# wirrell/SPART-python

Hardware: AMD Instinct MI355X
Metric: SPART spectra/sec (R_TOC+R_TOA+L_TOA) at batch 1M; achieved HBM GB/s vs peak (higher is better)
Workload: dtype f32

## Files before the change

### spart-python_amd/csrc/spart_kernels.h

```cpp
#pragma once

#include <type_traits>

#include "spart_math.h"

namespace spart {

constexpr int TILE = 256;
constexpr int NTILE = 8;
constexpr int NTILE_FULL = 9;
constexpr int MAX_NB = NWLS;

__device__ __forceinline__ void xcd_map(unsigned b, int& tile, int64_t& ck) {
  tile = (int)((b >> 3) & 7u);
  ck = (int64_t)(b >> 6) * 8 + (b & 7u);
}
inline unsigned xcd_grid(int64_t nchunk) { return (unsigned)(((nchunk + 7) / 8) * 64); }

struct ParamPtrs {
  const double* p[NPARAM];
  const double* rho_th;
  const double* tau_th;
  const double* lidf;
  int nlayers;
// ... 13 lines not shown
  const int si = threadIdx.x & 31, i0 = threadIdx.x >> 5;
  const unsigned lane_off = ((unsigned)i0 * (unsigned)Bp + (unsigned)si) * (unsigned)sizeof(T);
  if (si < nsub) {
#pragma unroll
    for (int k = 0; k < NCONST / 8; ++k) {
      const T* row = blk + (int64_t)(8 * k) * Bp;
      lds_c[si * NCONST + i0 + 8 * k] = *reinterpret_cast<const T*>(reinterpret_cast<const char*>(row) + lane_off);
    }
  }
}

template <typename T, int SUB>
__device__ __forceinline__ void stage_fetch(T (&r)[NCONST * SUB / TILE], const T* __restrict__ blk, int64_t Bp, int nsub) {
  constexpr int RP = TILE / SUB;
  static_assert(TILE % SUB == 0 && NCONST % RP == 0, "whole passes");
  const int si = threadIdx.x % SUB, i0 = threadIdx.x / SUB;
  const unsigned lane_off = ((unsigned)i0 * (unsigned)Bp + (unsigned)si) * (unsigned)sizeof(T);
  if (si < nsub) {
#pragma unroll
    for (int k = 0; k < NCONST / RP; ++k) {
      const T* row = blk + (int64_t)(RP * k) * Bp;
      r[k] = *reinterpret_cast<const T*>(reinterpret_cast<const char*>(row) + lane_off);
    }
  }
}
template <typename T, int SUB>
__device__ __forceinline__ void stage_put(T* lds_c, const T (&r)[NCONST * SUB / TILE], int nsub) {
  constexpr int RP = TILE / SUB;
  const int si = threadIdx.x % SUB, i0 = threadIdx.x / SUB;
  if (si < nsub) {
#pragma unroll
    for (int k = 0; k < NCONST / RP; ++k) lds_c[si * NCONST + i0 + RP * k] = r[k];
  }
}

struct PreludeStore {
  float* cstF;
  double* cstD;
  double* atm;
  int64_t Bp, s;
  __device__ __forceinline__ void c(int i, double v) const {
    if (cstF) cstF[i * Bp + s] = (float)v;
    if (cstD) cstD[i * Bp + s] = v;
  }
  __device__ __forceinline__ void a(int i, double v) const {
    if (atm) atm[i * Bp + s] = v;
  }
  __device__ __forceinline__ void l(int, double) const {}
};

constexpr int PRELUDE_SIMD_WAVES = 3;
template <bool FAST, bool USER = false>
__global__ __launch_bounds__(256, PRELUDE_SIMD_WAVES) void k_prelude(ParamPtrs pp, int mask, int64_t B, int64_t Bp, float* __restrict__ cstF,
                                                 double* __restrict__ cstD, double* __restrict__ atm) {
  const int64_t base = (int64_t)blockIdx.x * blockDim.x;
  int64_t s = base + threadIdx.x;
  if (!FAST && (mask & PRE_CANOPY) && !(USER && pp.lidf)) {
    constexpr int NB = 32;
    __shared__ int cnt[NB], start[NB];
    __shared__ unsigned char perm[256];
    const int t = threadIdx.x;
    int bucket = NB - 1;
    if (s < B) {
      const double key = ::fabs(pp.p[16][s]) + ::fabs(pp.p[17][s]);
      const double q = key * (NB / 1.0);
      bucket = !(q < (double)(NB - 1)) ? NB - 1 : (q > 0.0 ? (int)q : 0);
    }
    if (t < NB) cnt[t] = 0;
    __syncthreads();
    const int pos = atomicAdd(&cnt[bucket], 1);
    __syncthreads();
    if (t == 0) {
      int acc = 0;
      for (int i = 0; i < NB; ++i) { start[i] = acc; acc += cnt[i]; }
    }
    __syncthreads();
    perm[start[bucket] + pos] = (unsigned char)t;
    __syncthreads();
    s = base + perm[t];
  }
  if (s >= B) return;
  double rho_th = pp.rho_th ? pp.rho_th[s] : 0.01;
  double tau_th = pp.tau_th ? pp.tau_th[s] : 0.01;
  PreludeStore out{cstF, cstD, atm, Bp, s};
  if (USER)
    sample_prelude_to<FAST, true>([&pp, s](int i) { return pp.p[i] ? pp.p[i][s] : 0.0; }, rho_th, tau_th, mask, out,
                                  pp.lidf ? pp.lidf + s * NLINCL : nullptr, pp.nlayers);
  else
    sample_prelude_to<FAST>([&pp, s](int i) { return pp.p[i] ? pp.p[i][s] : 0.0; }, rho_th, tau_th, mask, out);
}

static __global__ __launch_bounds__(256) void k_lidf(const double* __restrict__ a, const double* __restrict__ b, int64_t B,
                                              double* __restrict__ lidf) {
  int64_t s = (int64_t)blockIdx.x * blockDim.x + threadIdx.x;
  if (s >= B) return;
  double li[NLINCL];
  leaf_angles(a[s], b[s], li);
#pragma unroll
  for (int i = 0; i < NLINCL; ++i) lidf[s * NLINCL + i] = li[i];
}

template <typename T> __device__ __forceinline__ BandTab<T> load_tab(const T* __restrict__ tab, int i) {
  BandTab<T> t;
  t.kab = tab[TAB_KAB * NWL + i];
  t.kca = tab[TAB_KCA * NWL + i];
  t.kdm = tab[TAB_KDM * NWL + i];
  t.kw = tab[TAB_KW * NWL + i];
  t.ks = tab[TAB_KS * NWL + i];
  t.kant = tab[TAB_KANT * NWL + i];
  t.kcbc = tab[TAB_CBC * NWL + i];
  t.kprot = tab[TAB_PROT * NWL + i];
  t.talf = tab[TAB_TALF * NWL + i];
  t.t12 = tab[TAB_T12 * NWL + i];
  t.t21 = tab[TAB_T21 * NWL + i];
  t.g0 = tab[TAB_GSV0 * NWL + i];
  t.g1 = tab[TAB_GSV1 * NWL + i];
  t.g2 = tab[TAB_GSV2 * NWL + i];
  t.cbac = tab[TAB_CBAC * NWL + i];
  t.pw = tab[TAB_PW * NWL + i];
  t.rw = tab[TAB_RW * NWL + i];
  return t;
}

template <typename T, typename C> __device__ __forceinline__ CanopyPar<T> load_canopy(const C& c) {
  CanopyPar<T> cp;
  cp.sob = c[C_SOB]; cp.sof = c[C_SOF];
  cp.hbf = c[C_HBF]; cp.ks = c[C_KS]; cp.ko = c[C_KO]; cp.lai = c[C_LAI]; cp.lai2 = c[C_LAI2];
  cp.tss = c[C_TSS]; cp.too = c[C_TOO]; cp.Z = c[C_Z]; cp.hot = c[C_HOT]; cp.pso2w = c[C_PSO2W];
  return cp;
}

template <bool NT = false, typename T> __device__ __forceinline__ void store_row(T* row, unsigned byte_off, T v) {
  T* p = reinterpret_cast<T*>(reinterpret_cast<char*>(row) + byte_off);
  if (NT) __builtin_nontemporal_store(v, p);
  else *p = v;
}
inline bool nt_ok(int pitch_elems, size_t elem_size) { return ((size_t)pitch_elems * elem_size) % 128 == 0; }

template <typename T> struct MatPtrs {
  T *leaf_refl, *leaf_tran, *leaf_kchl, *soil_refl, *soil_dry, *rso, *rdo, *rsd, *rdd;
  const T* rdry_in;
  int pf, po;
};

template <typename T, int MAT, int FULL, bool NT = false>
__global__ __launch_bounds__(TILE, (sizeof(T) == 8 ? 3 : 1))
void k_bands(const T* __restrict__ tab, const T* __restrict__ cst, int64_t Bp, int64_t B, int chunk, MatPtrs<T> mat,
             T* __restrict__ bandsum) {
  int tile;
  int64_t ck;
  xcd_map(blockIdx.x, tile, ck);
  if (ck * chunk >= B) return;
  if (sizeof(T) == 8) stage_f64_tables();
  const int band = tile * TILE + threadIdx.x;
  const bool active = band < NEVAL;
  const bool thermal = band == NWL;
  const int ti = band < NWL ? band : NWL - 1;
  const BandTab<T> tb = load_tab(tab, ti);
  const int64_t s0 = ck * chunk;
  const int64_t s1 = (s0 + chunk < B) ? s0 + chunk : B;
  T sum_so = T(0), sum_do = T(0), sum_sd = T(0), sum_dd = T(0);
  unsigned off_f = (unsigned)band * (unsigned)sizeof(T), off_o = off_f;
  if (MAT) {
    const int64_t b0f = s0 * mat.pf, b0o = s0 * mat.po;
    if (mat.leaf_refl) mat.leaf_refl += b0f;
    if (mat.leaf_tran) mat.leaf_tran += b0f;
    if (mat.soil_refl) mat.soil_refl += b0f;
    if (mat.rso) mat.rso += b0f;
    if (mat.rdo) mat.rdo += b0f;
    if (mat.rsd) mat.rsd += b0f;
    if (mat.rdd) mat.rdd += b0f;
    if (mat.leaf_kchl) mat.leaf_kchl += b0o;
    if (mat.soil_dry) mat.soil_dry += b0o;
  }
  constexpr int SUB = 32;
  constexpr bool HOIST_FILM = sizeof(T) == 8;
  constexpr bool PINGPONG = sizeof(T) == 4 && MAT == 0;
  __shared__ __attribute__((aligned(16))) T lds_all[(PINGPONG ? 2 : 1) * SUB * NCONST + (PINGPONG ? NCONST : 0)];
  T stg[NCONST * SUB / TILE];
  int cur = 0;
  if (PINGPONG) {
    const int n0 = (int)((s1 - s0 < SUB) ? (s1 - s0) : SUB);
    stage_fetch<T, SUB>(stg, cst + s0, Bp, n0);
    stage_put<T, SUB>(lds_all, stg, n0);
    __syncthreads();
  }
  for (int64_t sb = s0; sb < s1; sb += SUB) {
  const int nsub = (int)((s1 - sb < SUB) ? (s1 - sb) : SUB);
  T* const lds_c = lds_all + cur * (SUB * NCONST);
  const int nnext = (int)((s1 - sb - SUB < SUB) ? (s1 - sb - SUB) : SUB);
  if (PINGPONG) {
    if (nnext > 0) stage_fetch<T, SUB>(stg, cst + sb + SUB, Bp, nnext);
  } else {
    __syncthreads();
    stage_constants<T>(lds_c, cst + sb, Bp, nsub);
    __syncthreads();
  }
  bool film_same = false;
  T tw1s = T(0);
  if (HOIST_FILM) {
    const int l = threadIdx.x & 63;
    const T f0 = lds_c[C_FILM2L];
    const T fl = lds_c[(l < nsub ? l : 0) * NCONST + C_FILM2L];
    film_same = __all(fl == f0) != 0;
    if (film_same) tw1s = soil_tw1<T>(tb, f0);
  }
  constexpr bool AHEAD = MAT == 0 && sizeof(T) == 4;
  static_assert(AHEAD == PINGPONG, "the look-ahead read relies on the padding of lds_all");
  int lane0 = 0;
  if (AHEAD) {
    SPART_KEEP_BRANCH(lane0);
    lane0 &= ~3;
  }
  T lc[9];
#pragma unroll
  for (int i = 0; i < 9; ++i) lc[i] = lds_c[i];
  constexpr bool COMMON = sizeof(T) == 4 && MAT == 0 && FULL == 1;
  bool common = false;
  T tw1c = T(0);
  if (COMMON) {
    const int l = threadIdx.x & 63;
    const T* cl = lds_c + (l < nsub ? l : 0) * NCONST;
    common = __all(cl[C_FILM2L] == lds_c[C_FILM2L] && cl[C_CBC] == T(0) && cl[C_PROT] == T(0)) != 0;
    if (common) tw1c = soil_tw1<T>(tb, lds_c[C_FILM2L]);
  }
  constexpr bool VOTES = sizeof(T) == 4 && MAT == 0;
  unsigned long long j2_mask = ~0ull;
  if constexpr (VOTES) {
    const int l = threadIdx.x & 63;
    const T* cl = lds_c + (l < nsub ? l : 0) * NCONST;
    j2_mask = __ballot(sail_j2_possible(cl[C_KSL], cl[C_LAI]) || sail_j2_possible(cl[C_KOL], cl[C_LAI]));
  }
  auto sample_loop = [&](auto common_tag) __attribute__((always_inline)) {
  constexpr bool FAST = decltype(common_tag)::value;
  for (int si = 0; si < nsub; ++si) {
    const int64_t s = sb + si;
    const T* c = lds_c + si * NCONST + lane0;
    T refl, tran, absb, K;
    static_assert(C_CAB == 0 && C_NM1 == 8, "lc[] = constants 0..8 in leaf_band's argument order");
    if (!AHEAD) {
#pragma unroll
      for (int i = 0; i < 9; ++i) lc[i] = c[i];
    }
    leaf_band<T, !FAST>(tb, lc[0], lc[1], lc[2], lc[3], lc[4], lc[5], lc[6], lc[7], lc[8], refl, tran, absb, K);
    if (AHEAD) {
      const T* cn = c + NCONST;
#pragma unroll
      for (int i = 0; i < 9; ++i) lc[i] = cn[i];
    }
    T rho = refl, tau = tran, ab = absb;
    if (tile == NTILE - 1) {
      rho = thermal ? c[C_RHO_TH] : refl;
      tau = thermal ? c[C_TAU_TH] : tran;
      ab = thermal ? (T(1) - c[C_RHO_TH] - c[C_TAU_TH]) : absb;
    }
    if (MAT && active) {
      if (mat.leaf_refl) store_row<NT>(mat.leaf_refl, off_f, rho);
      if (mat.leaf_tran) store_row<NT>(mat.leaf_tran, off_f, tau);
      if (!thermal && mat.leaf_kchl) store_row<NT>(mat.leaf_kchl, off_o, (K > T(0)) ? divx(c[C_CAB] * tb.kab, K) : T(0));
    }
    const CanopyPar<T> cp = load_canopy<T>(c);
    const CanopyCore<T> core = canopy_core_l<T>(cp, rho, tau, ab, c[C_KSL], c[C_KOL], !VOTES || ((j2_mask >> si) & 1) != 0);
    T rdry = (MAT == 2) ? mat.rdry_in[s * mat.po + ti] : soil_dry<T>(tb, c[C_F1], c[C_F2], c[C_F3]);
    T fm[7] = {c[C_FM0], c[C_FM1], c[C_FM2], c[C_FM3], c[C_FM4], c[C_FM5], c[C_FM6]};
    T rwet, tw1;
    if (FAST) tw1 = tw1c;
    else if (HOIST_FILM && film_same) tw1 = tw1s;
    else tw1 = soil_tw1<T>(tb, c[C_FILM2L]);
    soil_band_tw<T>(tb, rdry, c[C_WET], fm, c[C_FMSUM], tw1, rwet);
    if (MAT && active) {
      if (mat.soil_refl) store_row<NT>(mat.soil_refl, off_f, rwet);
      if (!thermal && mat.soil_dry) store_row<NT>(mat.soil_dry, off_o, rdry);
    }
    constexpr bool SUM_ONLY = FULL == 1 && MAT == 0 && sizeof(T) == 4;
    T rso, rdo, rsd, rdd;
    if (SUM_ONLY) {
      sum_so += canopy_soil_sum<T>(cp, core, rwet, c[C_TSTO]);
    } else {
      canopy_soil<T>(cp, core, rwet, rso, rdo, rsd, rdd);
      if (FULL == 2) {
        sum_so += rso; sum_do += rdo; sum_sd += rsd; sum_dd += rdd;
      } else if (FULL == 1) {
        sum_so += (rso + rdo) + (rsd + rdd);
      }
    }
    if (MAT) {
      if (active) {
        if (mat.rso) store_row<NT>(mat.rso, off_f, rso);
        if (mat.rdo) store_row<NT>(mat.rdo, off_f, rdo);
        if (mat.rsd) store_row<NT>(mat.rsd, off_f, rsd);
        if (mat.rdd) store_row<NT>(mat.rdd, off_f, rdd);
      }
      constexpr int TH_WAVE = (NWL % TILE) / 64, TH_LANE = (NWL % TILE) % 64;
      if (tile == NTILE - 1 && (int)(threadIdx.x >> 6) == TH_WAVE) {
        const unsigned pad = off_f + (unsigned)((TH_LANE + 1) * (int)sizeof(T));
        T* arrs[7] = {mat.leaf_refl, mat.leaf_tran, mat.soil_refl, mat.rso, mat.rdo, mat.rsd, mat.rdd};
        const T vals[7] = {rho, tau, rwet, rso, rdo, rsd, rdd};
        const int l = threadIdx.x & 63;
#pragma unroll
        for (int q = 0; q < 7; ++q) {
          const T v = __shfl(vals[q], TH_LANE, 64);
          if (arrs[q]) {
            store_row(arrs[q], pad, v);
            store_row(arrs[q], pad + 64u * (unsigned)sizeof(T), v);
            if (l < NWLT - 1 - 128) store_row(arrs[q], pad + 128u * (unsigned)sizeof(T), v);
          }
        }
      }
      off_f += (unsigned)mat.pf * (unsigned)sizeof(T);
      off_o += (unsigned)mat.po * (unsigned)sizeof(T);
    }
  }
  };
  if constexpr (COMMON) {
    if (common) sample_loop(std::true_type{});
    else sample_loop(std::false_type{});
  } else {
    sample_loop(std::false_type{});
  }
  if (PINGPONG) {
    if (nnext > 0) stage_put<T, SUB>(lds_all + (cur ^ 1) * (SUB * NCONST), stg, nnext);
    __syncthreads();
    cur ^= 1;
  }
  }
  if (FULL == 2) {
    T* bs = bandsum + (ck * (NTILE * TILE) + band) * 4;
    bs[0] = sum_so; bs[1] = sum_do; bs[2] = sum_sd; bs[3] = sum_dd;
  } else if (FULL == 1) {
    bandsum[ck * (NTILE * TILE) + band] = sum_so;
  }
}

template <typename T> struct LdsCol {
  const T* p;
  __device__ __forceinline__ T operator[](int i) const { return p[i * 64]; }
};


constexpr int COL_WAVES = 4;
constexpr int COLUMNS_SIMD_WAVES = 4;

template <typename TG, typename TO, typename TR>
__global__ __launch_bounds__(64 * COL_WAVES, COLUMNS_SIMD_WAVES) void k_columns(
    const TG* __restrict__ tab, const TG* __restrict__ cst, const double* __restrict__ atm, int64_t Bp,
    const int* __restrict__ band0, const int* __restrict__ band1, const double* __restrict__ frac,
    const double* __restrict__ coef, const double* __restrict__ econv, int nb, const TR* __restrict__ rdry_in, int po, int64_t B,
    TO* __restrict__ R_TOC, TO* __restrict__ R_TOA, TO* __restrict__ L_TOA, TO* __restrict__ o_rsoil, TO* __restrict__ o_La) {
  __shared__ TG lds_c[NCONST_USED * 64];
  __shared__ double lds_a[NATM_USED * 64];
  __shared__ double lds_k[COL_WAVES * 64];
  if (sizeof(TG) == 8) stage_f64_tables();
  const int lane = threadIdx.x & 63;
  const int wave = __builtin_amdgcn_readfirstlane((int)(threadIdx.x >> 6));
  const int64_t s0 = (int64_t)blockIdx.x * 64;
  const int64_t s = s0 + lane;
  const bool ok = s < B;
  const int64_t sc = ok ? s : B - 1;
  for (int i = wave; i < NCONST_USED; i += COL_WAVES) lds_c[i * 64 + lane] = cst[(int64_t)i * Bp + sc];
  for (int i = wave; i < NATM_USED; i += COL_WAVES) lds_a[i * 64 + lane] = atm[(int64_t)i * Bp + sc];
  __syncthreads();
  const LdsCol<TG> c{lds_c + lane};
  const LdsCol<double> a{lds_a + lane};
  const bool want_soil = o_rsoil != nullptr;
  for (int j = wave; j < nb; j += COL_WAVES) {
    const int b0 = band0[j], b1 = band1[j];
    const double f = frac[j];
    const double kv = coef[(size_t)(lane < NCOEF ? lane : NCOEF - 1) * nb + j];
    double y0[5], y1[5];
#pragma unroll 1
    for (int e = 0; e < 2; ++e) {
      if (e == 1 && b1 == b0) break;
      const int band = e ? b1 : b0;
      const bool thermal = band == NWL;
      const int ti = band < NWL ? band : NWL - 1;
      const BandTab<TG> tb = load_tab(tab, ti);
      TG refl, tran, absb, K;
      leaf_band<TG>(tb, c[C_CAB], c[C_CCA], c[C_CDM], c[C_CW], c[C_CS], c[C_CANT], c[C_CBC], c[C_PROT], c[C_NM1], refl,
                    tran, absb, K);
      const TG rho = thermal ? c[C_RHO_TH] : refl;
      const TG tau = thermal ? c[C_TAU_TH] : tran;
      const TG ab = thermal ? (TG(1) - c[C_RHO_TH] - c[C_TAU_TH]) : absb;
      const CanopyPar<TG> cp = load_canopy<TG>(c);
      const CanopyCore<TG> core = canopy_core<TG>(cp, rho, tau, ab);
      const TG rdry = rdry_in ? (TG)rdry_in[sc * po + ti] : soil_dry<TG>(tb, c[C_F1], c[C_F2], c[C_F3]);
      TG fm[7] = {c[C_FM0], c[C_FM1], c[C_FM2], c[C_FM3], c[C_FM4], c[C_FM5], c[C_FM6]};
      TG rwet;
      soil_band<TG>(tb, rdry, c[C_WET], fm, c[C_FMSUM], c[C_FILM2L], rwet);
      TG rso, rdo, rsd, rdd;
      canopy_soil<TG>(cp, core, rwet, rso, rdo, rsd, rdd);
      const double v[5] = {(double)rso, (double)rdo, (double)rsd, (double)rdd, (double)rwet};
#pragma unroll
      for (int q = 0; q < 5; ++q) {
        if (e == 0) y0[q] = v[q];
        y1[q] = v[q];
      }
    }
    double v[5];
#pragma unroll
    for (int q = 0; q < 5; ++q) v[q] = y0[q] + (y1[q] - y0[q]) * f;
    double* kw = lds_k + wave * 64;
    kw[lane] = kv;
    __builtin_amdgcn_fence(__ATOMIC_RELEASE, "wavefront");
    __builtin_amdgcn_wave_barrier();
    __builtin_amdgcn_fence(__ATOMIC_ACQUIRE, "wavefront");
    const SmacOut so = smac_band_c(a, [kw](int r) { return kw[r]; });
    const double La = a[A_LAF] * econv[j];
    double rtoc, rtoa, ltoa;
    toc_to_toa(so, v[0], v[1], v[3], v[2], La, rtoc, rtoa, ltoa);
    if (ok) {
      const int64_t o = s * nb + j;
      R_TOC[o] = (TO)rtoc;
      R_TOA[o] = (TO)rtoa;
      L_TOA[o] = (TO)ltoa;
      if (want_soil) o_rsoil[o] = (TO)v[4];
      if (o_La) o_La[o] = (TO)La;
    }
  }
}

template <typename TO, typename TR>
__global__ __launch_bounds__(64 * COL_WAVES, COLUMNS_SIMD_WAVES) void k_columns_srf(
    const double* __restrict__ tab, const double* __restrict__ cst, const double* __restrict__ atm, int64_t Bp,
    const int* __restrict__ deal, const int* __restrict__ sup_start, const int* __restrict__ sup_ev,
    const double* __restrict__ sup_q, const double* __restrict__ sup_Q, const double* __restrict__ coef,
    const double* __restrict__ econv, int nb, const TR* __restrict__ rdry_in, int po, int64_t B, TO* __restrict__ R_TOC,
    TO* __restrict__ R_TOA, TO* __restrict__ L_TOA, TO* __restrict__ o_rso, TO* __restrict__ o_rdo, TO* __restrict__ o_rsd,
    TO* __restrict__ o_rdd) {
  __shared__ double lds_c[NCONST_USED * 64];
  __shared__ double lds_a[NATM_USED * 64];
  __shared__ double lds_k[COL_WAVES * 64];
  stage_f64_tables();
  const int lane = threadIdx.x & 63;
  const int wave = __builtin_amdgcn_readfirstlane((int)(threadIdx.x >> 6));
  const int64_t s = (int64_t)blockIdx.x * 64 + lane;
  const bool ok = s < B;
  const int64_t sc = ok ? s : B - 1;
  for (int i = wave; i < NCONST_USED; i += COL_WAVES) lds_c[i * 64 + lane] = cst[(int64_t)i * Bp + sc];
  for (int i = wave; i < NATM_USED; i += COL_WAVES) lds_a[i * 64 + lane] = atm[(int64_t)i * Bp + sc];
  __syncthreads();
  const int j = deal[blockIdx.y * COL_WAVES + wave];
  if (j < 0) return;
  const int e0 = sup_start[j], e1 = sup_start[j + 1];
  double acc_so = 0.0, acc_do = 0.0, acc_sd = 0.0, acc_dd = 0.0;
#pragma unroll 1
  for (int e = e0; e < e1; ++e) {
    int lo = lane;
    SPART_KEEP_BRANCH(lo);
    const LdsCol<double> c{lds_c + lo};
    const int band = sup_ev[e];
    const double q = sup_q[e];
    const bool thermal = band == NWL;
    const int ti = band < NWL ? band : NWL - 1;
    const BandTab<double> tb = load_tab(tab, ti);
    double refl, tran, absb, K;
    leaf_band<double>(tb, c[C_CAB], c[C_CCA], c[C_CDM], c[C_CW], c[C_CS], c[C_CANT], c[C_CBC], c[C_PROT], c[C_NM1], refl,
                      tran, absb, K);
    const double rho = thermal ? c[C_RHO_TH] : refl;
    const double tau = thermal ? c[C_TAU_TH] : tran;
    const double ab = thermal ? (1.0 - c[C_RHO_TH] - c[C_TAU_TH]) : absb;
    const CanopyPar<double> cp = load_canopy<double>(c);
    const CanopyCore<double> core = canopy_core<double>(cp, rho, tau, ab);
    const double rdry = rdry_in ? (double)rdry_in[sc * po + ti] : soil_dry<double>(tb, c[C_F1], c[C_F2], c[C_F3]);
    double fm[7] = {c[C_FM0], c[C_FM1], c[C_FM2], c[C_FM3], c[C_FM4], c[C_FM5], c[C_FM6]};
    double rwet;
    soil_band<double>(tb, rdry, c[C_WET], fm, c[C_FMSUM], c[C_FILM2L], rwet);
    double rso, rdo, rsd, rdd;
    canopy_soil<double>(cp, core, rwet, rso, rdo, rsd, rdd);
    acc_so = __builtin_fma(q, rso, acc_so);
    acc_do = __builtin_fma(q, rdo, acc_do);
    acc_sd = __builtin_fma(q, rsd, acc_sd);
    acc_dd = __builtin_fma(q, rdd, acc_dd);
  }
  const LdsCol<double> a{lds_a + lane};
  const double Q = sup_Q[j];
  const double v_so = acc_so / Q, v_do = acc_do / Q, v_sd = acc_sd / Q, v_dd = acc_dd / Q;
  double* kw = lds_k + wave * 64;
  kw[lane] = coef[(size_t)(lane < NCOEF ? lane : NCOEF - 1) * nb + j];
  __builtin_amdgcn_fence(__ATOMIC_RELEASE, "wavefront");
  __builtin_amdgcn_wave_barrier();
  __builtin_amdgcn_fence(__ATOMIC_ACQUIRE, "wavefront");
  const SmacOut so = smac_band_c(a, [kw](int r) { return kw[r]; });
  const double La = a[A_LAF] * econv[j];
// ... 178 lines not shown
```

### spart-python_amd/csrc/spart_math.h

```cpp
#pragma once

#include <cmath>
#include <cstdint>

#if defined(__HIPCC__)
#include <hip/hip_runtime.h>
#define SPART_HD __host__ __device__ __forceinline__
#else
#define SPART_HD inline
#endif

#if defined(__clang__)
#define SPART_NO_CONTRACT _Pragma("clang fp contract(off)")
#else
#define SPART_NO_CONTRACT
#endif

#if defined(__HIP_DEVICE_COMPILE__)
#define SPART_WAVE_ANY(c) (__builtin_amdgcn_ballot_w64(c) != 0)
#define SPART_KEEP_BRANCH(x) asm volatile("" : "+v"(x))
#else
#define SPART_WAVE_ANY(c) (c)
#define SPART_KEEP_BRANCH(x) ((void)0)
#endif
// ... 183 lines not shown
  }
  static SPART_HD double exp_finish(double k, double r) {
    const int ki = (int)k;
    const double t = s_f64_exp_tab[ki & (F64_EXP_TAB - 1)];
    double p = spart_horner(1.0 / 24.0, r, 1.0 / 6.0);
    p = __builtin_fma(p, r, 0.5);
    p = __builtin_fma(p, r * r, r);
    return __builtin_ldexp(__builtin_fma(t, p, t), ki >> 8);
  }
  static SPART_HD double exp(double x) {
    x = __builtin_fmax(x, -800.0);
    const double k = __builtin_rint(x * 369.32993046757463);
    double r = __builtin_fma(-k, 0.0027076061737716373, x);
    r = __builtin_fma(-k, 2.9064910585985925e-13, r);
    return exp_finish(k, r);
  }
  static SPART_HD double exp2(double x) {
    const double t = x * 256.0;
    const double k = __builtin_rint(t);
    return exp_finish(k, (t - k) * 0.0027076061740622863);
  }
  static SPART_HD double log(double x) {
    const unsigned long long u = (unsigned long long)__double_as_longlong(x);
    const unsigned hi = (unsigned)(u >> 32);
    const int e = (int)(hi >> 20) - 1023;
    const unsigned i = (hi >> 12) & (unsigned)(F64_LOG_TAB - 1);
    const double m = __longlong_as_double((long long)((u & 0x000FFFFFFFFFFFFFull) | 0x3FF0000000000000ull));
    const double R = s_f64_log_tab[2 * i], L = s_f64_log_tab[2 * i + 1];
    const double z = __builtin_fma(m, R, -1.0);
    double q = spart_horner(-1.0 / 6.0, z, 0.2);
    q = spart_horner(q, z, -0.25);
    q = spart_horner(q, z, 1.0 / 3.0);
    q = __builtin_fma(q, z, -0.5);
    const double p = __builtin_fma(z * z, q, z);
    return __builtin_fma((double)e, 0.6931471805599453, L + p);
  }
#else
  static SPART_HD double exp_poly(double x) { return ::exp(x); }
  static SPART_HD double exp(double x) { return ::exp(x); }
  static SPART_HD double exp2(double x) { return ::exp2(x); }
  static SPART_HD double log(double x) { return ::log(x); }
#endif
  static SPART_HD double sqrt(double x) {
#if defined(__HIP_DEVICE_COMPILE__) && defined(SPART_FAST_MATH)
    const double y0 = __builtin_amdgcn_rsq(x + 1e-300);
    const double g = x * y0;
    const double e = __builtin_fma(-g, y0, 1.0);
    return __builtin_fma(g * 0.5, e, g);
#else
    return ::sqrt(x);
#endif
  }
  static SPART_HD double rcp(double x) {
#if defined(__HIP_DEVICE_COMPILE__) && defined(SPART_FAST_MATH)
    const double r = __builtin_amdgcn_rcp(x);
    return __builtin_fma(__builtin_fma(-x, r, 1.0), r, r);
#else
    return 1.0 / x;
#endif
  }
  static SPART_HD double log1p(double x) {
#if defined(SPART_FAST_MATH)
    if (x < 0.1) {
      double s = x * rcp(2.0 + x), s2 = s * s;
      double p = horner_c(1.0 / 13.0, s2, 1.0 / 11.0);
      p = horner_c(p, s2, 1.0 / 9.0);
      p = horner_c(p, s2, 1.0 / 7.0);
      p = horner_c(p, s2, 0.2);
      p = horner_c(p, s2, 1.0 / 3.0);
      p = p * s2 + 1.0;
      return 2.0 * s * p;
    }
    return log(1.0 + x);
#else
    return ::log1p(x);
#endif
  }
  static SPART_HD double omen_taylor(double z) {
    double p = -1.0 / 40320.0;
    p = p * z + 1.0 / 5040.0;
    p = p * z - 1.0 / 720.0;
    p = p * z + 1.0 / 120.0;
    p = p * z - 1.0 / 24.0;
    p = p * z + 1.0 / 6.0;
    p = p * z - 0.5;
    p = p * z + 1.0;
    return z * p;
  }
  static SPART_HD double one_minus_exp_neg(double z) {
#if defined(SPART_FAST_MATH)
    if (::fabs(z) < 0.02) return omen_taylor(z);
    return 1.0 - exp(-z);
#else
    return -::expm1(-z);
#endif
  }
  static SPART_HD double one_minus_exp_neg_poly(double z) {
#if defined(SPART_FAST_MATH)
    return (::fabs(z) < 0.02) ? omen_taylor(z) : 1.0 - exp_poly(-z);
#else
    return -::expm1(-z);
#endif
  }
  static SPART_HD double one_minus_exp_neg(double z, double ez) {
#if defined(SPART_FAST_MATH)
    return (::fabs(z) < 0.02) ? omen_taylor(z) : 1.0 - ez;
#else
    (void)ez;
    return -::expm1(-z);
#endif
  }
  static SPART_HD double fabs(double x) { return ::fabs(x); }
  static SPART_HD double fmax(double a, double b) { return ::fmax(a, b); }
  static SPART_HD double tiny() { return 1e-300; }
};

template <typename T> SPART_HD T divx(T a, T b) { return a * Mx<T>::rcp(b); }

template <typename T> struct SailJ;
template <> struct SailJ<float> {
  static constexpr float THRESH = 0.06f;
  static SPART_HD float poly(float d) {
    return 1.0f + d * (-0.5f + d * (0.166666667f + d * (-0.0416666667f + d * 8.33333333e-3f)));
  }
};
template <> struct SailJ<double> {
  static constexpr double THRESH = 2e-3;
  static SPART_HD double poly(double d) {
    return 1.0 + d * (-0.5 + d * (1.0 / 6.0 + d * (-1.0 / 24.0 + d * (1.0 / 120.0 - d * (1.0 / 720.0)))));
  }
};
template <typename T> SPART_HD T sail_j1_d(T L, T tk, T e1, T d, T id) {
  T v = L * (tk - e1) * id;
  const bool small = Mx<T>::fabs(d) < SailJ<T>::THRESH;
  if (SPART_WAVE_ANY(small)) {
    SPART_KEEP_BRANCH(d);
    v = small ? L * tk * SailJ<T>::poly(d) : v;
  }
  return v;
}
template <typename T> SPART_HD T sail_j1_a(T L, T tk, T e1, T d, T ia) {
  T v = L * Mx<T>::fabs(tk - e1) * ia;
  const bool small = Mx<T>::fabs(d) < SailJ<T>::THRESH;
  if (SPART_WAVE_ANY(small)) {
    SPART_KEEP_BRANCH(d);
    v = small ? L * tk * SailJ<T>::poly(d) : v;
  }
  return v;
}
template <typename T> SPART_HD T sail_j2_d(T L, T tk, T e1, T kpm, T ikpm, bool maybe_small = true) {
  T v = (T(1) - tk * e1) * ikpm;
  if (maybe_small) {
    T d = kpm * L;
    if (SPART_WAVE_ANY(d < SailJ<T>::THRESH)) {
      SPART_KEEP_BRANCH(d);
      v = (d < SailJ<T>::THRESH) ? L * SailJ<T>::poly(d) : v;
    }
  }
  return v;
}
constexpr float SAIL_J2_GUARD_F32 = 0.07f;
SPART_HD bool sail_j2_possible(float kl, float L) { return !(kl >= SAIL_J2_GUARD_F32) || !(L > 0.0f); }

template <typename T> struct E3c;
template <> struct E3c<float> {
  static constexpr int GD = E3_G_DEG_F32, WD = E3_W_DEG_F32;
  static constexpr float PSCALE = 2.0f;
  static SPART_HD const float* gt() { return E3_G_F32; }
  static SPART_HD const float* pt() { return E3_P_F32; }
  static SPART_HD const float* qt() { return E3_Q_F32; }
};
#if defined(__HIPCC__)
static_assert(E3_G_DEG_F64 == 12 && E3_W_DEG_F64 == 6, "tables below list the coefficients one by one");
#define SPART_L13(a) {a[0], a[1], a[2], a[3], a[4], a[5], a[6], a[7], a[8], a[9], a[10], a[11], a[12]}
#define SPART_L7(a) {a[0], a[1], a[2], a[3], a[4], a[5], a[6]}
static __device__ __constant__ double c_E3_G_F64[13] = SPART_L13(E3_G_F64);
#define SPART_L7X2(a) {2 * a[0], 2 * a[1], 2 * a[2], 2 * a[3], 2 * a[4], 2 * a[5], 2 * a[6]}
static __device__ __constant__ double c_E3_P_F64[7] = SPART_L7X2(E3_P_F64);
static __device__ __constant__ double c_E3_Q_F64[7] = SPART_L7(E3_Q_F64);
#endif
template <> struct E3c<double> {
  static constexpr int GD = E3_G_DEG_F64, WD = E3_W_DEG_F64;
#if defined(__HIP_DEVICE_COMPILE__)
  static constexpr double PSCALE = 1.0;
#else
  static constexpr double PSCALE = 2.0;
#endif
#if defined(__HIP_DEVICE_COMPILE__)
  static SPART_HD spart_cdp gt() { return spart_fresh(c_E3_G_F64); }
  static SPART_HD spart_cdp pt() { return spart_fresh(c_E3_P_F64); }
  static SPART_HD spart_cdp qt() { return spart_fresh(c_E3_Q_F64); }
#else
  static SPART_HD const double* gt() { return E3_G_F64; }
  static SPART_HD const double* pt() { return E3_P_F64; }
  static SPART_HD const double* qt() { return E3_Q_F64; }
#endif
};

#if defined(__HIPCC__)
SPART_HD double horner_uniform(double p, double x, double c) { return spart_horner(p, x, c); }
#else
SPART_HD double horner_uniform(double p, double x, double c) { return p * x + c; }
#endif
SPART_HD float horner_uniform(float p, float x, float c) { return p * x + c; }

template <typename T> SPART_HD void plate_tau(T K, T& tau, T& u) {
  using C = E3c<T>;
  T x = (K < Mx<T>::tiny()) ? Mx<T>::tiny() : K;
  const bool small = x < T(1);
  T tl, ul;
  if (small) {
    const auto cg = C::gt();
    T g = cg[C::GD];
#pragma unroll
    for (int i = C::GD - 1; i >= 0; --i) g = horner_uniform(g, x, cg[i]);
    ul = x * (g + x * Mx<T>::log(x));
    tl = T(1) - ul;
  } else {
    const auto cp = C::pt(), cq = C::qt();
    T pn = C::PSCALE * cp[0], qn = cq[0];
#pragma unroll
    for (int i = 1; i <= C::WD; ++i) {
      pn = horner_uniform(pn, x, C::PSCALE * cp[i]);
      qn = horner_uniform(qn, x, cq[i]);
    }
    tl = Mx<T>::exp(-x) * pn * Mx<T>::rcp((x + T(3)) * qn);
    ul = T(1) - tl;
  }
  tau = tl;
  u = ul;
}

inline double calculate_tav(double alpha, double nr) {
  const double rd = PI / 180.0;
  double n2 = nr * nr, n_p = n2 + 1, nm = n2 - 1;
  double a = (nr + 1) * (nr + 1) / 2;
  double k = -(n2 - 1) * (n2 - 1) / 4;
  double sa = std::sin(alpha * rd);
  double b1 = 0;
  if (alpha != 90) b1 = std::sqrt((sa * sa - n_p / 2) * (sa * sa - n_p / 2) + k);
  double b2 = sa * sa - n_p / 2;
  double b = b1 - b2;
  double b3 = b * b * b, a3 = a * a * a;
  double ts = (k * k / (6 * b3) + k / b - b / 2) - (k * k / (6 * a3) + k / a - a / 2);
  double tp1 = -2 * n2 * (b - a) / (n_p * n_p);
  double tp2 = -2 * n2 * n_p * std::log(b / a) / (nm * nm);
  double tp3 = n2 * (1 / b - 1 / a) / 2;
  double tp4 = 16 * n2 * n2 * (n2 * n2 + 1) * std::log((2 * n_p * b - nm * nm) / (2 * n_p * a - nm * nm)) /
               (n_p * n_p * n_p * nm * nm);
  double tp5 = 16 * n2 * n2 * n2 * (1 / (2 * n_p * b - nm * nm) - 1 / (2 * n_p * a - nm * nm)) / (n_p * n_p * n_p);
  double tp = tp1 + tp2 + tp3 + tp4 + tp5;
  return (ts + tp) / (2 * sa * sa);
}

inline double wl_solar_at(int i) {
  return i < NWL ? 400.0 + i : (i < NWL + 126 ? 2500.0 + 100.0 * (i - NWL) : 16000.0 + 1000.0 * (i - NWL - 126));
}

inline void interp_support(double x, int& e0, int& e1, double& frac) {
  auto eval_of = [](int grid_idx) { return grid_idx < NWL ? grid_idx : NWL; };
  int i0 = 0;
  while (i0 + 1 < NWLS - 1 && wl_solar_at(i0 + 1) <= x) ++i0;
  int i1 = i0 + 1;
  double f = (x - wl_solar_at(i0)) / (wl_solar_at(i1) - wl_solar_at(i0));
  if (!(f > 0.0)) f = 0.0;
  if (f > 1.0) f = 1.0;
  e0 = eval_of(i0);
  e1 = f > 0.0 ? eval_of(i1) : e0;
  frac = f;
}

enum TabRow {
  TAB_KAB = 0, TAB_KCA, TAB_KDM, TAB_KW, TAB_KS, TAB_KANT, TAB_CBC, TAB_PROT,
  TAB_TALF, TAB_T12, TAB_T21,
  TAB_GSV0, TAB_GSV1, TAB_GSV2,
  TAB_CBAC, TAB_PW, TAB_RW,
  NTAB
};

template <typename T> struct BandTab {
  T kab, kca, kdm, kw, ks, kant, kcbc, kprot, talf, t12, t21, g0, g1, g2, cbac, pw, rw;
};

enum ConstIdx {
  C_CAB = 0, C_CCA, C_CDM, C_CW, C_CS, C_CANT, C_CBC, C_PROT, C_NM1, C_RHO_TH, C_TAU_TH,
  C_F1, C_F2, C_F3, C_WET, C_FM0, C_FM1, C_FM2, C_FM3, C_FM4, C_FM5, C_FM6, C_FMSUM, C_FILM2L,
  C_SOB, C_SOF, C_HBF, C_KS, C_KO, C_LAI, C_LAI2, C_TSS, C_TOO, C_Z, C_HOT, C_PSO2W,
  C_KSL, C_KOL, C_TSTO, C_RSV3,
  NCONST
};
constexpr int NCONST_USED = C_KSL;
static_assert(NCONST == 40, "constant block is 40 values");

enum AtmIdx {
  A_US = 0, A_UV, A_M, A_PEQ, A_PA, A_AOT, A_CKSI, A_KSID, A_LAF,
  A_LOGPEQ, A_LOGM, A_LOGO3M, A_LOGH2OM,
  A_RSV,
  NATM = 16
};
constexpr int NATM_USED = A_RSV;

template <typename T, bool PRO = true>
SPART_HD void leaf_band(const BandTab<T>& tb, T cab, T cca, T cdm, T cw, T cs, T cant, T cbc, T prot, T nm1,
                        T& refl, T& tran, T& absb, T& Kall) {
  T K = cab * tb.kab + cca * tb.kca + cdm * tb.kdm + cw * tb.kw + cs * tb.ks + cant * tb.kant;
  if (PRO) K = K + cbc * tb.kcbc + prot * tb.kprot;
  else (void)cbc, (void)prot;
// ... 832 lines not shown
```

Baseline: 105.9 million.

## Split tail wave's 18 live bands across three sample phases

In the f32 sum-only band kernel, the last tile's fourth wave has only 18 live lanes (the last one thermal). This change remaps that wave so its 64 lanes cover the 18 bands in three phases, each handling about a third of the 32-sample stage, and shares partial results through an LDS deposit buffer. It also precomputes the thermal absorptance into LDS and marks the small-argument SAIL J2 branch as unlikely. This targets the critical-path wave that otherwise loops over all samples with most lanes idle, at the cost of extra LDS, per-lane index arithmetic and a serial reduction over the deposited values.

```diff
diff --git a/spart-python_amd/csrc/spart_kernels.h b/spart-python_amd/csrc/spart_kernels.h
--- a/spart-python_amd/csrc/spart_kernels.h
+++ b/spart-python_amd/csrc/spart_kernels.h
@@ -189,7 +189,26 @@
   xcd_map(blockIdx.x, tile, ck);
   if (ck * chunk >= B) return;
   if (sizeof(T) == 8) stage_f64_tables();
-  const int band = tile * TILE + threadIdx.x;
+  constexpr int SUB = 32;
+  constexpr bool TAIL3 = sizeof(T) == 4 && MAT == 0 && FULL == 1;
+  constexpr int TAIL_BAND0 = (NTILE - 1) * TILE + 3 * 64, TAIL_N = NEVAL - TAIL_BAND0, TAIL_P = (SUB + 2) / 3;
+  static_assert(NEVAL - 7 * TILE - 3 * 64 == 18 && TAIL_N == 18 && TAIL_BAND0 + TAIL_N - 1 == NWL, "18 live lanes, the last one thermal");
+  static_assert(3 * TAIL_N <= 64 && 3 * TAIL_P >= SUB && TAIL_P == 11, "three phases fit one wave and cover a stage");
+  const bool tailw = TAIL3 && tile == NTILE - 1 && __builtin_amdgcn_readfirstlane((int)(threadIdx.x >> 6)) == 3;
+  const int slot = tile * TILE + threadIdx.x;
+  auto tail_lane = [&](int& b, int& p) __attribute__((always_inline)) {
+    int l = threadIdx.x & 63;
+    SPART_KEEP_BRANCH(l);
+    l = l < 3 * TAIL_N ? l : 3 * TAIL_N - 1;
+    p = l / TAIL_N;
+    b = l - p * TAIL_N;
+  };
+  int band = slot;
+  if (tailw) {
+    int b, p;
+    tail_lane(b, p);
+    band = TAIL_BAND0 + b;
+  }
   const bool active = band < NEVAL;
   const bool thermal = band == NWL;
   const int ti = band < NWL ? band : NWL - 1;
@@ -210,10 +229,13 @@
     if (mat.leaf_kchl) mat.leaf_kchl += b0o;
     if (mat.soil_dry) mat.soil_dry += b0o;
   }
-  constexpr int SUB = 32;
   constexpr bool HOIST_FILM = sizeof(T) == 8;
   constexpr bool PINGPONG = sizeof(T) == 4 && MAT == 0;
-  __shared__ __attribute__((aligned(16))) T lds_all[(PINGPONG ? 2 : 1) * SUB * NCONST + (PINGPONG ? NCONST : 0)];
+  constexpr int LDS_PAD = TAIL3 ? 3 * TAIL_P + 1 - SUB : 1;
+  static_assert(!TAIL3 || (PINGPONG && SUB + LDS_PAD >= 3 * TAIL_P + 1), "every tail-wave read stays inside lds_all");
+  __shared__ __attribute__((aligned(16))) T lds_all[(PINGPONG ? 2 : 1) * SUB * NCONST + (PINGPONG ? LDS_PAD * NCONST : 0)];
+  __shared__ T dep[TAIL3 ? 3 * TAIL_P * TAIL_N : 1];
+  static_assert(sizeof(dep) <= 2376, "the tail wave's deposit: 33 samples x 18 values");
   T stg[NCONST * SUB / TILE];
   int cur = 0;
   if (PINGPONG) {
@@ -226,6 +248,13 @@
   const int nsub = (int)((s1 - sb < SUB) ? (s1 - sb) : SUB);
   T* const lds_c = lds_all + cur * (SUB * NCONST);
   const int nnext = (int)((s1 - sb - SUB < SUB) ? (s1 - sb - SUB) : SUB);
+  const int npass = (tailw && nsub > TAIL_P) ? TAIL_P : nsub;
+  int tail_c0 = 0;
+  if (tailw) {
+    int b, p;
+    tail_lane(b, p);
+    tail_c0 = p * (TAIL_P * NCONST);
+  }
   if (PINGPONG) {
     if (nnext > 0) stage_fetch<T, SUB>(stg, cst + sb + SUB, Bp, nnext);
   } else {
@@ -248,10 +277,11 @@
   if (AHEAD) {
     SPART_KEEP_BRANCH(lane0);
     lane0 &= ~3;
+    if (TAIL3) lane0 += tail_c0;
   }
   T lc[9];
 #pragma unroll
-  for (int i = 0; i < 9; ++i) lc[i] = lds_c[i];
+  for (int i = 0; i < 9; ++i) lc[i] = lds_c[(TAIL3 ? tail_c0 : 0) + i];
   constexpr bool COMMON = sizeof(T) == 4 && MAT == 0 && FULL == 1;
   bool common = false;
   T tw1c = T(0);
@@ -268,9 +298,16 @@
     const T* cl = lds_c + (l < nsub ? l : 0) * NCONST;
     j2_mask = __ballot(sail_j2_possible(cl[C_KSL], cl[C_LAI]) || sail_j2_possible(cl[C_KOL], cl[C_LAI]));
   }
+  if constexpr (TAIL3) {
+    if (tailw) {
+      j2_mask |= (j2_mask >> TAIL_P) | (j2_mask >> (2 * TAIL_P));
+      const int l = threadIdx.x & 63;
+      if (l < SUB) lds_c[l * NCONST + C_RSV3] = T(1) - lds_c[l * NCONST + C_RHO_TH] - lds_c[l * NCONST + C_TAU_TH];
+    }
+  }
   auto sample_loop = [&](auto common_tag) __attribute__((always_inline)) {
   constexpr bool FAST = decltype(common_tag)::value;
-  for (int si = 0; si < nsub; ++si) {
+  for (int si = 0; si < npass; ++si) {
     const int64_t s = sb + si;
     const T* c = lds_c + si * NCONST + lane0;
     T refl, tran, absb, K;
@@ -286,10 +323,10 @@
       for (int i = 0; i < 9; ++i) lc[i] = cn[i];
     }
     T rho = refl, tau = tran, ab = absb;
-    if (tile == NTILE - 1) {
+    if (TAIL3 ? tailw : tile == NTILE - 1) {
       rho = thermal ? c[C_RHO_TH] : refl;
       tau = thermal ? c[C_TAU_TH] : tran;
-      ab = thermal ? (T(1) - c[C_RHO_TH] - c[C_TAU_TH]) : absb;
+      ab = thermal ? (TAIL3 ? c[C_RSV3] : T(1) - c[C_RHO_TH] - c[C_TAU_TH]) : absb;
     }
     if (MAT && active) {
       if (mat.leaf_refl) store_row<NT>(mat.leaf_refl, off_f, rho);
@@ -312,7 +349,14 @@
     constexpr bool SUM_ONLY = FULL == 1 && MAT == 0 && sizeof(T) == 4;
     T rso, rdo, rsd, rdd;
     if (SUM_ONLY) {
-      sum_so += canopy_soil_sum<T>(cp, core, rwet, c[C_TSTO]);
+      const T v = canopy_soil_sum<T>(cp, core, rwet, c[C_TSTO]);
+      sum_so += v;
+      if (TAIL3 && tailw) {
+        int sj = si, b, p;
+        asm volatile("" : "+s"(sj));
+        tail_lane(b, p);
+        dep[(p * TAIL_P + sj) * TAIL_N + b] = v;
+      }
     } else {
       canopy_soil<T>(cp, core, rwet, rso, rdo, rsd, rdd);
       if (FULL == 2) {
@@ -355,6 +399,13 @@
   } else {
     sample_loop(std::false_type{});
   }
+  if constexpr (TAIL3) {
+    if (tailw && nsub > TAIL_P) {
+      int b, p;
+      tail_lane(b, p);
+      for (int j = TAIL_P; j < nsub; ++j) sum_so += dep[j * TAIL_N + b];
+    }
+  }
   if (PINGPONG) {
     if (nnext > 0) stage_put<T, SUB>(lds_all + (cur ^ 1) * (SUB * NCONST), stg, nnext);
     __syncthreads();
@@ -362,10 +413,10 @@
   }
   }
   if (FULL == 2) {
-    T* bs = bandsum + (ck * (NTILE * TILE) + band) * 4;
+    T* bs = bandsum + (ck * (NTILE * TILE) + slot) * 4;
     bs[0] = sum_so; bs[1] = sum_do; bs[2] = sum_sd; bs[3] = sum_dd;
   } else if (FULL == 1) {
-    bandsum[ck * (NTILE * TILE) + band] = sum_so;
+    bandsum[ck * (NTILE * TILE) + slot] = (TAIL3 && tailw && (int)(threadIdx.x & 63) >= TAIL_N) ? T(0) : sum_so;
   }
 }
 
diff --git a/spart-python_amd/csrc/spart_math.h b/spart-python_amd/csrc/spart_math.h
--- a/spart-python_amd/csrc/spart_math.h
+++ b/spart-python_amd/csrc/spart_math.h
@@ -359,7 +359,7 @@
   T v = (T(1) - tk * e1) * ikpm;
   if (maybe_small) {
     T d = kpm * L;
-    if (SPART_WAVE_ANY(d < SailJ<T>::THRESH)) {
+    if (__builtin_expect(SPART_WAVE_ANY(d < SailJ<T>::THRESH), 0)) {
       SPART_KEEP_BRANCH(d);
       v = (d < SailJ<T>::THRESH) ? L * SailJ<T>::poly(d) : v;
     }
```

Result: no change. 105.4 million (-0.5%).
